# Fancomi2017/InstanceFusion

Hardware: AMD Instinct MI355X
Metric: frames/s + ms/frame (ICP|fuse|instance) at 640x480, 5M surfels, 1/2/4/8 GPU (higher is better)
Workload: dtype f32; 1 GPU; 5000000-surfel map, 640x480 synthetic RGBD stream, 3-level ICP+RGB + surfel fuse + canned-mask instance votes with superpixel refinement; surfels_live=4734799, surfel_slots=4734799, map_order=random, parallelism=replicas x1, loop_frames=90

## Files before the change

include/ifx_c_api.h:

```cpp
#ifndef IFX_C_API_H_
#define IFX_C_API_H_

#include <stdint.h>

#ifdef __cplusplus
extern "C" {
#endif

#define IFX_NUM_INSTANCES 96
#define IFX_VOTE_FLOATS 48

enum {
    IFX_OK = 0,
    IFX_E_INVALID = -1,
    IFX_E_HIP = -2,
    IFX_E_CAPACITY = -3,
    IFX_E_STATE = -4
};

typedef struct ifx_config {
    int32_t width, height;
    float fx, fy, cx, cy;
    int32_t time_delta;
    float confidence;
// ... 53 lines not shown
int ifx_owner_ids_resume(ifx_t* h);
int ifx_owner_knn_export(ifx_t* h, void** d_points, void** d_labels, int* n);
int ifx_owner_knn_vote(ifx_t* h, const void* d_all_points, const void* d_all_labels, int n_all, int own_offset);
int ifx_map_seq(ifx_t* h, uint32_t* out, int max_n);
int ifx_map_bounding_boxes(ifx_t* h, int bbox_type, float ratio, float* boxes96x6, float* ground_normal3, float* gc_matrix16, float* inst_matrix96x16,
                           int32_t* ground_votes648);
int ifx_instance_point_cloud(ifx_t* h, int bbox_type, int32_t* counts96, int inst, float* out10, int max_records);
int ifx_view_list_stats(ifx_t* h, int32_t* out4);
int ifx_sync(ifx_t* h);
int ifx_get_pose(ifx_t* h, float* out_pose16);
int ifx_tick(ifx_t* h);
int ifx_trajectory(ifx_t* h, float* out_poses16, int max_frames);
int ifx_tracker_diag(ifx_t* h, float* diag8);
int ifx_tracker_fallbacks(ifx_t* h);
int ifx_tracker_range_exceeded(ifx_t* h);

int ifx_set_loop_closure(ifx_t* h, int enable, int count_thresh, float err_thresh, float cov_thresh);
int ifx_loop_closure_diag(ifx_t* h, float* out24);
typedef int (*ifx_loop_closure_cb)(ifx_t* h, const float* lc24, void* user);
int ifx_set_loop_closure_callback(ifx_t* h, ifx_loop_closure_cb cb, void* user);
int ifx_sample_graph_model(ifx_t* h, float* out_xyzt, int max_n);
int ifx_loop_closure_constraints(ifx_t* h, float* src3, float* dst3, int32_t* times, int max_n);
int ifx_set_deformation(ifx_t* h, const float* graph16, int n_nodes, int is_fern);
int ifx_adopt_estimated_pose(ifx_t* h);

typedef int (*ifx_fern_cb)(ifx_t* h, void* user);
int ifx_set_fern_callback(ifx_t* h, ifx_fern_cb cb, void* user);
int ifx_adopt_pose(ifx_t* h, const float* pose16);
int ifx_fern_frame(ifx_t* h, uint8_t* img_rgb, float* verts4, float* norms4, uint8_t* inst_rgb);
int ifx_fern_frame_async(ifx_t* h);
// ... 184 lines not shown
```

instancefusion_amd/__init__.py:

```python
from __future__ import annotations

import ctypes as C
import functools
import os

import numpy as np

_HERE = os.path.dirname(os.path.abspath(__file__))
LIB_PATH = os.environ.get("IFX_LIB") or os.path.join(_HERE, "libifx.so")
HEADER_PATH = os.path.join(os.path.dirname(_HERE), "include", "ifx_c_api.h")

NUM_INSTANCES = 96
VOTE_FLOATS = 48


class IfxError(RuntimeError):
    pass


class IfxConfig(C.Structure):
    _fields_ = [
        ("width", C.c_int32), ("height", C.c_int32),
        ("fx", C.c_float), ("fy", C.c_float), ("cx", C.c_float), ("cy", C.c_float),
        ("time_delta", C.c_int32), ("confidence", C.c_float), ("depth_cut", C.c_float),
# ... 87 lines not shown
    "ifx_prefetch_frame_device": (C.c_int, [_P, _P, _P]),
    "ifx_hint_next_frame_device": (C.c_int, [_P, _P, _P]),
    "ifx_hint_next_frame": (C.c_int, [_P, _P, _P]),
    "ifx_lookahead_stats": (C.c_int, [_P, _P, C.c_int]),
    "ifx_view_list_stats": (C.c_int, [_P, _P]),
    "ifx_map_bounding_boxes": (C.c_int, [_P, C.c_int, C.c_float, _P, _P, _P, _P, _P]),
    "ifx_instance_point_cloud": (C.c_int, [_P, C.c_int, _P, C.c_int, _P, C.c_int]),
    "ifx_sync": (C.c_int, [_P]),
    "ifx_get_pose": (C.c_int, [_P, _P]),
    "ifx_tick": (C.c_int, [_P]),
    "ifx_trajectory": (C.c_int, [_P, _P, C.c_int]),
    "ifx_tracker_diag": (C.c_int, [_P, _P]),
    "ifx_tracker_fallbacks": (C.c_int, [_P]),
    "ifx_build_pyramids": (C.c_int, [_P, _P, _P, _P, _P, _P, _P, C.POINTER(Pyramids)]),
    "ifx_tracker_range_exceeded": (C.c_int, [_P]),
    "ifx_hot_records_stale": (C.c_int, [_P]),
    "ifx_set_loop_closure": (C.c_int, [_P, C.c_int, C.c_int, C.c_float, C.c_float]),
    "ifx_loop_closure_diag": (C.c_int, [_P, _P]),
    "ifx_set_loop_closure_callback": (C.c_int, [_P, _P, _P]),
    "ifx_sample_graph_model": (C.c_int, [_P, _P, C.c_int]),
    "ifx_loop_closure_constraints": (C.c_int, [_P, _P, _P, _P, C.c_int]),
    "ifx_set_deformation": (C.c_int, [_P, _P, C.c_int, C.c_int]),
    "ifx_adopt_estimated_pose": (C.c_int, [_P]),
    "ifx_set_fern_callback": (C.c_int, [_P, _P, _P]),
    "ifx_adopt_pose": (C.c_int, [_P, _P]),
    "ifx_fern_frame": (C.c_int, [_P, _P, _P, _P, _P]),
    "ifx_fern_frame_async": (C.c_int, [_P]),
    "ifx_fern_frame_fetch": (C.c_int, [_P, _P, _P, _P, _P]),
    "ifx_track_maps": (C.c_int, [_P, _P, _P, _P, _P, _P, _P, _P, _P]),
    "ifx_map_view": (C.c_int, [_P, C.POINTER(SoaView)]),
# ... 814 lines not shown
        out = np.zeros((max_frames, 16), np.float32)
        n = self._chk(self.L.ifx_trajectory(self.handle, _ptr(out), max_frames), "ifx_trajectory")
        return out[:n].reshape(n, 4, 4).copy()

    def tracker_diag(self):
        out = np.zeros(8, np.float32)
        self._chk(self.L.ifx_tracker_diag(self.handle, _ptr(out)), "ifx_tracker_diag")
        return out

    def tracker_fallbacks(self):
        return self._chk(self.L.ifx_tracker_fallbacks(self.handle), "ifx_tracker_fallbacks")

    def tracker_range_exceeded(self):
        return self._chk(self.L.ifx_tracker_range_exceeded(self.handle), "ifx_tracker_range_exceeded")

    def set_loop_closure(self, enable=True, count_thresh=35000, err_thresh=5e-5, cov_thresh=1e-5):
        self._chk(self.L.ifx_set_loop_closure(self.handle, int(enable), int(count_thresh), err_thresh, cov_thresh), "ifx_set_loop_closure")

    def loop_closure_diag(self):
        out = np.zeros(24, np.float32)
        self._chk(self.L.ifx_loop_closure_diag(self.handle, _ptr(out)), "ifx_loop_closure_diag")
        return dict(ran=bool(out[0]), inactive_pixels=int(out[1]), icp_error=float(out[2]), icp_count=float(out[3]), cov_ok=bool(out[4]),
                    accepted=bool(out[5]), est_pose=out[6:22].reshape(4, 4).copy(), cov_max=float(out[22]), candidates=int(out[23]))

    def set_loop_closure_callback(self, fn):
        if fn is None:
            self._lc_cb = None
            self._chk(self.L.ifx_set_loop_closure_callback(self.handle, None, None), "ifx_set_loop_closure_callback")
            return

# ... 481 lines not shown
```

instancefusion_amd/csrc/ifx_api.hip:

```cpp
#include <climits>
#include "ifx_ctx.h"
#include <string.h>
#include <stdio.h>
#include <algorithm>

int ifx_tracker_external_pose(ifx* h, const float* d_pose16, float weight_mult);
int ifx_tracker_set_weight(ifx* h, float weight_mult);
int ifx_compact_enqueue(ifx* h, int refresh_ids);

void hs_invalidate_view(ifx* h);
static std::string g_err;
extern "C" const char* ifx_global_error(void) { return g_err.c_str(); }
extern "C" const char* ifx_last_error(ifx_t* h) { return h ? h->err.c_str() : g_err.c_str(); }

hipEvent_t ifx_event_get(ifx* h)
{
    if (!h->event_pool.empty()) { hipEvent_t e = h->event_pool.back(); h->event_pool.pop_back(); return e; }
    hipEvent_t e;
    hipEventCreate(&e);
    return e;
}
void ifx_ktime_begin(ifx* h, const char* name, hipEvent_t* a)
{
    (void)name;
// ... 338 lines not shown
    else if (s == "ff_rounds") h->opt_ff_rounds = value;
    else if (s == "gn_persist_blocks") { if (value < 1) return IFX_E_INVALID; ifx_drop_tracked(h); h->opt_gn_persist_blocks = value; }
    else if (s == "gn_persist") {
        if (value < 0 || value > 7) { h->err = "gn_persist is a mask of pyramid levels (0..7)"; return IFX_E_INVALID; }
        ifx_drop_tracked(h);
        h->opt_gn_persist = value;
    }
    else if (s == "gn_spin_limit" || s == "gn_fault") {
        if (value < 0) return IFX_E_INVALID;
        ifx_drop_tracked(h);
        HIPCHK(h, hipStreamSynchronize(h->stream));
        HIPCHK(h, hipMemcpy((char*)h->d_state + (s == "gn_fault" ? offsetof(DevState, gn_fault) : offsetof(DevState, gn_spin_limit)), &value, sizeof(int), hipMemcpyHostToDevice));
    }
    else if (s == "gn_prologue") { ifx_drop_tracked(h); h->opt_gn_prologue = value ? 1 : 0; }
    else if (s == "rgb_cand") { ifx_drop_tracked(h); h->opt_rgb_cand = value ? 1 : 0; }
    else if (s == "raster_lds") h->opt_raster_lds = value;
    else if (s == "raster_earlyz") h->opt_raster_earlyz = value;
    else if (s == "pyramid" || s == "fast_odom" || s == "so3" || s == "icp_weight_x1000") {
        if (h->hint_rgb || h->slot[h->tick & 1].for_tick == h->tick) { h->err = "tracker options cannot change while a frame is announced ahead"; return IFX_E_STATE; }
        ifx_drop_tracked(h);
        if (s == "pyramid") h->cfg.pyramid = value ? 1 : 0;
        else if (s == "fast_odom") h->cfg.fast_odom = value ? 1 : 0;
        else if (s == "so3") h->cfg.so3 = value ? 1 : 0;
        else { if (value < 0 || value > 100000) { h->err = "icp_weight_x1000 must be in [0, 100000]"; return IFX_E_INVALID; } h->cfg.icp_weight = value / 1000.f; }
    }
    else { h->err = "unknown option " + s; return IFX_E_INVALID; }
    return IFX_OK;
}

__global__ void k_frame_result(DevState* __restrict__ st, FrameResult* __restrict__ out, float* __restrict__ traj_slot)
// ... 765 lines not shown
extern "C" int ifx_tracker_fallbacks(ifx_t* h)
{
    if (!h) return IFX_E_INVALID;
    int r = ifx_sync(h);
    return r ? r : h->h_result->gn_timeout;
}

extern "C" int ifx_hot_records_stale(ifx_t* h)
{
    if (!h) return IFX_E_INVALID;
    HIPCHK(h, hipStreamSynchronize(h->stream));
    int v = 0;
    HIPCHK(h, hipMemcpy(&v, &h->d_state->hot_stale, sizeof(int), hipMemcpyDeviceToHost));
    return v;
}
extern "C" int ifx_tracker_range_exceeded(ifx_t* h)
{
    if (!h) return IFX_E_INVALID;
    int r = ifx_sync(h);
    if (r) return r;
    if (h->stream_c) HIPCHK(h, hipStreamSynchronize(h->stream_c));
    if (h->stream_b) HIPCHK(h, hipStreamSynchronize(h->stream_b));
    std::vector<const DevState*> sts;
    sts.push_back(h->d_state);
    if (h->d_m2m) sts.push_back(h->d_m2m);
    if (h->d_cam_trk) sts.push_back(h->d_cam_trk);
    for (const FrameSlot& f : h->slot) if (f.so3) sts.push_back(f.so3);
    long long total = 0;
    for (const DevState* d : sts) {
        int v = 0;
// ... 396 lines not shown
```

instancefusion_amd/csrc/ifx_ctx.h:

```cpp
#pragma once
#include <hip/hip_runtime.h>
#include <stdint.h>
#include <string>
#include <vector>
#include <map>
#include "../../include/ifx_c_api.h"
#include "ifx_dev.h"

#ifndef IFX_LIST_SEGS
#define IFX_LIST_SEGS 8
#endif

struct DevState {
    float pose[16];
    float pose_inv[16];
    float last_pose[16];
    float weighting;
    int dense_enough;
    int count;
    int n_dead;
    int n_new;
    int overflow;
    unsigned int r_max_bits;
    float Rprev[9], tprev[3], Rprev_inv[9];
// ... 30 lines not shown
    int vl_scans;
    unsigned int vl_n[2];
    unsigned int vl_seg_n[2 * IFX_LIST_SEGS], vl_seg_off[2 * IFX_LIST_SEGS];
    long long dbg[8];
    alignas(64) int gn_res[2];
    unsigned int gn_ticket;
    int gn_pad[13];
    double gn_acc[2 * IFX_ACC_REPL * IFX_ACC_STRIDE];
    double gn_acc2[2 * 2 * IFX_ACC_REPL * IFX_ACC_STRIDE];
    alignas(64) int gn_res2[2 * 16];
    alignas(64) unsigned int gn_bar[4 * 32 * 16];
    int gn_timeout;
    int gn_abort;
    int gn_done_seq;
    int gn_spin_limit, gn_fault;
    alignas(64) double gnp_acc[2 * 2 * IFX_ACC_REPL * IFX_ACC_STRIDE];
    alignas(64) int gnp_res[2 * 16];
    alignas(64) double gnp_RRt[2][16];
};

struct IdMap { const uint32_t* seq; int own_n; };
__device__ __forceinline__ int idmap_slot(const IdMap& m, int count, int id)
{
    if (m.own_n <= 0) return (id > 0 && id < count) ? id : -1;
    if (id == 0) return -1;
    int lo = 0, hi = count - 1;
    while (lo <= hi) {
        const int mid = (lo + hi) >> 1;
        const unsigned int v = m.seq[mid];
        if (v == (unsigned int)id) return mid;
        if (v < (unsigned int)id) lo = mid + 1; else hi = mid - 1;
    }
    return -1;
// ... 228 lines not shown
    std::vector<int> oseg_cmp, oseg_bbox, oseg_class;
    hipEvent_t oseg_ev = nullptr;
    int32_t* oseg_rec = nullptr;
    size_t oseg_rec_cap = 0, oseg_rec_bytes = 0;
    int oseg_root = -1, oseg_form = 0, oseg_M = 0, oseg_maxn = 0;
    float oseg_thr = 0.f;
    const char* oseg_who = "";
    void* d_kexp = nullptr;
    int gn_begin_folded = 0;
    int labels_stale_all = 1;
    int opt_raster_lds = 0;
    int opt_view_blocks = 0, opt_clean_blocks = 0, opt_index_blocks = 0;
    int icp_resident_blocks = 1024;
    int opt_res_blocks = 0;
    int opt_rgb_cand = 1;
    int opt_icp_blocks = 0;
    int opt_raster_tiles = -1;
    int map_external = 0;
    int lc_enable = 0, lc_count_thresh = 35000;
    float lc_err_thresh = 5e-5f, lc_cov_thresh = 1e-5f;
    DevState* d_m2m = nullptr;
    Pyr m2m;
    float *old_vertex = nullptr, *old_normal = nullptr;
    uint8_t *old_image = nullptr, *old_inst = nullptr;
    uint16_t* old_time = nullptr;
    float *act_vertex = nullptr, *act_normal = nullptr;
    uint8_t *act_image = nullptr, *act_inst = nullptr;
    uint16_t* act_time = nullptr;
    size_t lc_half = 0;
    int own_tracked_tick = 0;
// ... 206 lines not shown
```

instancefusion_amd/csrc/ifx_track.hip:

```cpp
#include "ifx_ctx.h"
#include <math.h>
#include <string.h>


#define BIL_R 6
#define BIL_BX 32
#define BIL_BY 8
template <bool SHIFTED, bool XCLIP>
__device__ __forceinline__ void bil_window(const uint16_t (*tile)[BIL_BX + 2 * BIL_R + 3], const unsigned char* s_mapx, const unsigned char* s_mapy, int x, int y, int bx, int by, int tx1,
                                           int ty1, unsigned int value, float& sum1, float& sum2)
{
    const float ss = 0.024691358f, sc = 0.000555556f;
    constexpr int D = BIL_R * 2 + 1;
    const float fv = (float)value;
    for (int cy = max(y - D / 2, 0); cy < ty1; ++cy) {
        const int ry = SHIFTED ? (int)s_mapy[cy - by + BIL_R + 1] : cy - by + BIL_R + 1;
        const float dy = (float)y - (float)cy, dy2 = dy * dy;
        float tv[D];
#pragma unroll
        for (int q = 0; q < D; q++) {
            const int col = x - D / 2 + q - bx + BIL_R + 1;
            tv[q] = (float)tile[ry][SHIFTED ? (int)s_mapx[col] : col];
        }
#pragma unroll
// ... 333 lines not shown
            const float g = c_gauss25[(ty - cy - 1) * 5 + (tx - cx - 1)];
            const float sf = din[cy * sw + cx];
            if (!(sf != sf)) { sumf += sf * g; cntf += (int)g; }
            const int si = iin[cy * sw + cx];
            if (si > 0) { sumi += si * g; cnti += (int)g; }
        }
    const float z = (float)(sumf / (float)cntf);
    o.depth[y * dw + x] = z;
    o.img[y * dw + x] = cnti ? (uint8_t)f2i_rz(sumi / (float)cnti) : (uint8_t)0;
    model_tail(st, x, y, dw, dh, res[0], res[1], z, o);
}


#define RED_THREADS 256
#define RED_WAVES (RED_THREADS / 64)

__device__ __forceinline__ double dpp_quad_sum_d(double v)
{
    {
        const int lo = __builtin_amdgcn_update_dpp(0, __double2loint(v), 0xB1, 0xF, 0xF, true), hi = __builtin_amdgcn_update_dpp(0, __double2hiint(v), 0xB1, 0xF, 0xF, true);
        v += __hiloint2double(hi, lo);
    }
    {
        const int lo = __builtin_amdgcn_update_dpp(0, __double2loint(v), 0x4E, 0xF, 0xF, true), hi = __builtin_amdgcn_update_dpp(0, __double2hiint(v), 0x4E, 0xF, 0xF, true);
        v += __hiloint2double(hi, lo);
    }
    return v;
}
template <int NV>
__device__ __forceinline__ void block_sum_exact(const double* acc, double* __restrict__ gacc, int rep)
// ... 95 lines not shown

struct KInv { double i0, i4, i2, i5; };
struct GnPro {
    int k;
    int icp, rgb;
    float icp_weight;
    float nfx, nfy, ncx, ncy;
    KInv ki;
};
__device__ __forceinline__ void gn_serial_lane(const double* s_sys, int icp, double* RRt, const float* Rp, const float* tp, float nfx, float nfy, float ncx, float ncy, const KInv& ki,
                                               float* Rc, float* tc, float* krk, float* kt);
__device__ __forceinline__ const float* gn_prologue(const DevState* __restrict__ st, const GnPro& g, double* __restrict__ rrt_out)
{
    __shared__ double s_psys[27];
    __shared__ float s_ppose[24];
    const int prev = (g.k - 1) & 1;
    const double* const icp_acc = st->gnp_acc + (size_t)(prev * 2) * IFX_ACC_REPL * IFX_ACC_STRIDE;
    const double* const rgb_acc = icp_acc + IFX_ACC_REPL * IFX_ACC_STRIDE;
    if (threadIdx.x < 27) {
        const int k = threadIdx.x;
        const double ti = acc_total(icp_acc, k), tr = acc_total(rgb_acc, k);
        const float oi = g.icp ? (float)ti : 0.f, orr = g.rgb ? (float)tr : 0.f;
        const double wgt = g.icp_weight;
        const double wa = wgt * wgt, wb = wgt;
        const bool is_b = (k == 6) | (k == 12) | (k == 17) | (k == 21) | (k == 24) | (k == 26);
        const double vi = (double)oi, vr = (double)orr;
        s_psys[k] = (g.icp && g.rgb) ? vr + (is_b ? wb : wa) * vi : (g.icp ? vi : vr);
    }
    const double* const rsrc = g.k == 1 ? st->resultRt : st->gnp_RRt[g.k & 1];
    double RRt[16];
    float Rp[9], tp[3];
// ... 195 lines not shown
        int s = 0;
        for (int wv = 0; wv < RED_WAVES; wv++) s += lds[wv][threadIdx.x];
        if (!FROM_STATE) partials[bid * 2 + threadIdx.x] = s;
        if (res_total && s) atomicAdd(&res_total[threadIdx.x], s);
    }
}
__global__ __launch_bounds__(RED_THREADS) void k_rgb_residual(const DevState* __restrict__ st, ResArgs ex, float minScale, const int16_t* __restrict__ dIdx,
                                                              const int16_t* __restrict__ dIdy, const float* __restrict__ lastDepth,
                                                              const float* __restrict__ nextDepth, const uint8_t* __restrict__ lastImage,
                                                              const uint8_t* __restrict__ nextImage, Corres8* __restrict__ corres, float maxDepthDelta,
                                                              int w, int h, int* __restrict__ partials)
{
    residual_body(blockIdx.x, gridDim.x, st, ex, minScale, dIdx, dIdy, lastDepth, nextDepth, lastImage, nextImage, corres, maxDepthDelta, w, h, partials);
}

template <bool PRO>
__device__ __forceinline__ void residual_cand_body(int bid, int nblk, const DevState* __restrict__ st, const CandEntry* __restrict__ cand, const unsigned int* __restrict__ cand_n,
                                                   const float* __restrict__ lastDepth, const float* __restrict__ nextDepth, const uint8_t* __restrict__ lastImage,
                                                   const uint8_t* __restrict__ nextImage, Corres8* __restrict__ corres, float maxDepthDelta, int w, int h,
                                                   int* __restrict__ res_total, const GnPro* pro, double* __restrict__ rrt_out)
{
    const int N = w * h;
    const int stride = nblk * RED_THREADS;
    int t = bid * RED_THREADS + threadIdx.x;
    const int n = min((int)cand_n[0], N);
    const CandEntry e0 = cand[t < N ? t : 0];
    CandEntry e1 = cand[t + stride < N ? t + stride : 0];
    int pix = t < n ? (int)min(e0.pixel, (uint32_t)(N - 1)) : 0;
    float d1 = nextDepth[pix];
    uint8_t ni = nextImage[pix];
    const float* kk = st->krkinv;
    const float* ktp = st->kt;
    if (PRO) { const float* sp = gn_prologue(st, *pro, rrt_out); kk = sp + 12; ktp = sp + 21; }
    float krk[9];
#pragma unroll
    for (int k = 0; k < 9; k++) krk[k] = kk[k];
    const float kt0 = ktp[0], kt1 = ktp[1], kt2 = ktp[2];
    int cnt = 0, sig = 0;
    while (t < n) {
        const int i = pix / w, j0 = pix - i * w;
// ... 5 lines not shown
        const int gj = c0 ? v0 * w + u0 : 0;
        const float d0 = lastDepth[gj];
        const uint8_t li = lastImage[gj];
        const int tn = t + stride, tnn = tn + stride;
        const int pixn = tn < n ? (int)min(e1.pixel, (uint32_t)(N - 1)) : 0;
        const float d1n = nextDepth[pixn];
        const uint8_t nin = nextImage[pixn];
        const CandEntry e2 = cand[tnn < N ? tnn : 0];
        Corres8 c;
        const bool hit = c0 & (d0 > 0) & (fabsf(td1 - d0) <= maxDepthDelta) & (li != 0);
        const float diff = (float)ni - (float)li;
        c.zx = hit ? (short)u0 : (short)-1; c.zy = hit ? (short)v0 : (short)-1;
        c.diff = hit ? diff : 0.f;
        cnt += hit ? 1 : 0;
        sig += hit ? (int)(diff * diff) : 0;
        corres[t] = c;
        t = tn; pix = pixn; d1 = d1n; ni = nin; e1 = e2;
    }
    __shared__ int lds[RED_WAVES][2];
    const int lane = threadIdx.x & 63, wid = threadIdx.x >> 6;
    cnt = wave_sum_i(cnt);
    sig = wave_sum_i(sig);
    if (lane == 0) { lds[wid][0] = cnt; lds[wid][1] = sig; }
    __syncthreads();
    if (threadIdx.x < 2) {
        int s = 0;
        for (int wv = 0; wv < RED_WAVES; wv++) s += lds[wv][threadIdx.x];
        if (s) atomicAdd(&res_total[threadIdx.x], s);
    }
}

struct PairArgs {
    const float *vmap_curr, *nmap_curr, *vmap_prev, *nmap_prev;
    float fx, fy, cx, cy, distThres, angleThres;
    float minScale, maxDepthDelta;
    const int16_t *dIdx, *dIdy;
    const float *lastDepth, *nextDepth;
    const uint8_t *lastImage, *nextImage;
    Corres8* corres;
    int w, h, nb_icp, nb_res;
    int check_skip;
};
#define IFX_PIN_S(x) asm volatile("" ::"s"(x))
template <bool CHECK_SKIP, bool PRO = false, bool LIST = false>
__global__ __launch_bounds__(RED_THREADS, 4) void k_icp_residual(const DevState* __restrict__ st, int nb_icp, int w, int h, double* __restrict__ gacc, int* __restrict__ gres, PairArgs a, GnPro g,
                                                              double* __restrict__ rrt_store, const CandEntry* __restrict__ cand, const unsigned int* __restrict__ cand_n)
{
    __builtin_assume(st != nullptr);
    if (CHECK_SKIP && st->skip) return;
    if ((int)blockIdx.x < nb_icp) {
        IcpArgs ia;
        icp_body<false, true, PRO>(blockIdx.x, nb_icp, st, ia, a.vmap_curr, a.nmap_curr, a.vmap_prev, a.nmap_prev, a.fx, a.fy, a.cx, a.cy, a.distThres, a.angleThres, w, h, gacc, &g,
                                   blockIdx.x == 0 ? rrt_store : nullptr);
    } else if (LIST) {
        residual_cand_body<PRO>(blockIdx.x - nb_icp, a.nb_res, st, cand, cand_n, a.lastDepth, a.nextDepth, a.lastImage, a.nextImage, a.corres, a.maxDepthDelta, w, h, gres, &g,
                                blockIdx.x == 0 ? rrt_store : nullptr);
    } else {
        ResArgs ra;
        residual_body<true, PRO>(blockIdx.x - nb_icp, a.nb_res, st, ra, a.minScale, a.dIdx, a.dIdy, a.lastDepth, a.nextDepth, a.lastImage, a.nextImage, a.corres, a.maxDepthDelta, w,
                                 h, nullptr, gres, &g, blockIdx.x == 0 ? rrt_store : nullptr);
    }
}
// ... 915 lines not shown
    int icp, rgb;
    float icp_weight, nfx, nfy, ncx, ncy;
    KInv ki;
    int check_skip;
    int final_iter;
    int end_run, commit;
    float weight_mult;
    unsigned int* lctr;
    int pro, pro_k;
};
template <bool CHECK_SKIP, bool LIST = false>
__global__ __launch_bounds__(RED_THREADS) void k_rgb_step_solve(DevState* st, int nb, int rgb, int w, int h, StepArgs a, const CandEntry* __restrict__ cand, const unsigned int* __restrict__ cand_n)
{
    __builtin_assume(st != nullptr);
    if (CHECK_SKIP && st->skip) return;
    const int par = a.pro_k & 1;
    int* const res_total = a.pro ? st->gnp_res + par * 16 : st->gn_res;
    unsigned int* const ticket = &st->gn_ticket;
    double* const icp_acc = a.pro ? st->gnp_acc + (size_t)(par * 2) * IFX_ACC_REPL * IFX_ACC_STRIDE : st->gn_acc;
    double* const rgb_acc = icp_acc + IFX_ACC_REPL * IFX_ACC_STRIDE;
    __shared__ int s_last;
    if (a.pro && blockIdx.x == 0) {
        double* const other = st->gnp_acc + (size_t)((1 - par) * 2) * IFX_ACC_REPL * IFX_ACC_STRIDE;
        if (threadIdx.x < 64) {
            const int kind = threadIdx.x >> 5, k = threadIdx.x & 31;
            if (k < 28 && range_exceeded7(kind, k, acc_total(other + (size_t)kind * IFX_ACC_REPL * IFX_ACC_STRIDE, k))) atomicAdd(&st->range_exceeded, 1);
        }
        __syncthreads();
        __hip_atomic_store(&other[threadIdx.x], 0.0, __ATOMIC_RELAXED, __HIP_MEMORY_SCOPE_AGENT);
        if (threadIdx.x < 2) __hip_atomic_store(&st->gnp_res[(1 - par) * 16 + threadIdx.x], 0, __ATOMIC_RELAXED, __HIP_MEMORY_SCOPE_AGENT);
    }
#ifdef IFX_STAMPS
    long long t0 = clock64();
#endif
    if (rgb) {
        if (LIST) rgb_step_cand_body(blockIdx.x, nb, a.corres, cand, cand_n, a.cloud, a.fx, a.fy, a.sobelScale, w, h, rgb_acc, res_total);
        else rgb_step_body(blockIdx.x, nb, a.corres, 0.f, nullptr, 0, a.cloud, a.fx, a.fy, a.dIdx, a.dIdy, a.sobelScale, w, h, rgb_acc, res_total);
    }
    if (a.pro == 1) return;
    asm volatile("s_waitcnt vmcnt(0)" ::: "memory");
    __syncthreads();
#ifdef IFX_STAMPS
    long long t1 = clock64();
#endif
    if (threadIdx.x == 0) {
// ... 497 lines not shown
    const int maxb = 1024;
    HIPCHK(h, hipMalloc(&p.acc, (3 * IFX_ACC_REPL * IFX_ACC_STRIDE * sizeof(double))));
    HIPCHK(h, hipMemset(p.acc, 0, (3 * IFX_ACC_REPL * IFX_ACC_STRIDE * sizeof(double))));
    {
        int cus = 0, dev = 0;
        hipGetDevice(&dev);
        hipDeviceGetAttribute(&cus, hipDeviceAttributeMultiprocessorCount, dev);
        int occ[4] = {0, 0, 0, 0};
        hipOccupancyMaxActiveBlocksPerMultiprocessor(&occ[0], k_gn_level<1>, RED_THREADS, 0);
        hipOccupancyMaxActiveBlocksPerMultiprocessor(&occ[1], k_gn_level<2>, RED_THREADS, 0);
        hipOccupancyMaxActiveBlocksPerMultiprocessor(&occ[2], k_gn_level<3>, RED_THREADS, 0);
        hipOccupancyMaxActiveBlocksPerMultiprocessor(&occ[3], k_gn_level<4>, RED_THREADS, 0);
        for (int q = 0; q < 4; q++) h->gn_max_blocks[q] = std::max(0, occ[q]) * std::max(0, cus);
        int occ_ir = 0;
        if (hipOccupancyMaxActiveBlocksPerMultiprocessor(&occ_ir, k_icp_residual<false, true>, RED_THREADS, 0) == hipSuccess && occ_ir > 0 && cus > 0) h->icp_resident_blocks = occ_ir * cus;
    }
    h->res_rows = std::max(maxb, cdiv(h->P, RED_THREADS) + 1);
    HIPCHK(h, hipMalloc(&h->res_partials, (size_t)h->res_rows * 2 * 4));
    HIPCHK(h, hipMalloc(&h->d_out29, 64 * 4));
    HIPCHK(h, hipMalloc(&h->d_ticket, 512));
    HIPCHK(h, hipMemset(h->d_ticket, 0, 512));
    p.res_partials = h->res_partials; p.ticket = h->d_ticket;
    for (int q = 0; q < 2; q++) {
        HIPCHK(h, hipMalloc(&h->slot[q].so3, sizeof(DevState)));
        HIPCHK(h, hipMemset(h->slot[q].so3, 0, sizeof(DevState)));
    }
    ifx_bind_slot(h, 0);
    return IFX_OK;
}

// ... 29 lines not shown
        hipFree(h->d_cam_trk); hipFree(h->cam_so3_acc); hipFree(h->cam_so3_ticket);
        h->d_cam_trk = nullptr;
    }
    free_m2m(h);
    hipFree(h->d_graph); hipFree(h->d_sample); hipFree(h->d_cons); hipFree(h->d_project); hipFree(h->d_fern); hipFree(h->d_inst_gt);
    if (h->h_fern) hipHostFree(h->h_fern);
    if (h->ev_fern) hipEventDestroy(h->ev_fern);
    hipFree(h->pyr.acc); hipFree(h->res_partials); hipFree(h->d_out29); hipFree(h->d_ticket);
}

static inline int rgb_cand_blocks(const ifx* h, int n, int level, bool step)
{
    const int per_thread = 8 >> std::min(level, 2), opt = step ? h->opt_rgb_blocks : h->opt_res_blocks;
    const int b = opt > 0 ? std::min(opt, cdiv(n, RED_THREADS)) : cdiv(n, RED_THREADS * per_thread * (step ? RED_IT_RGB : 1));
    return std::max(1, b);
}
static inline int red_blocks(ifx* h, int n, int it = RED_IT)
{
    int b = cdiv(n, RED_THREADS * it);
    const int cap = h->opt_icp_blocks > 0 ? h->opt_icp_blocks : std::max(456, std::min(1024, h->P / 2048));
    if (b > cap) b = cap;
    if (b < 1) b = 1;
    return b;
}

int ifx_tracker_init_first(ifx* h)
{
    Pyr& p = h->pyr;
    LAUNCH(h, "intensity", dim3(cdiv(h->P, 256)), dim3(256), k_intensity, h->rgb, 3, h->P, p.lastnext_img[0]);
    for (int i = 0; i + 1 < IFX_NUM_PYRS; i++)
// ... 175 lines not shown
            if (iterations[i] <= 0) continue;
            if (persist_q[i] >= 0) { if (seen_two_launch) pro = false; }
            else {
                seen_two_launch = true;
                const int n = p.w[i] * p.h[i];
                const int blocks = (icp ? red_blocks(h, n) : 0) + (cand_run ? rgb_cand_blocks(h, n, i, false) : rgb ? std::min(std::min(cdiv(n, RED_THREADS * RED_IT), h->res_rows), h->opt_res_blocks > 0 ? h->opt_res_blocks : (1 << 30)) : 0);
                small = small && blocks <= h->opt_gn_prologue_blocks;
                if (small) n_pro += iterations[i];
            }
        }
        if (n_pro < 2) pro = false;
    }
    int persist_iters = 0;
    int tail_k = 0;
    char* const stb = (char*)st;
    auto gnp_acc_of = [&](int par) { return (double*)(stb + offsetof(DevState, gnp_acc)) + (size_t)(par * 2) * IFX_ACC_REPL * IFX_ACC_STRIDE; };
    auto gnp_res_of = [&](int par) { return (int*)(stb + offsetof(DevState, gnp_res)) + par * 16; };
    auto gnp_rrt_of = [&](int par) { return (double*)(stb + offsetof(DevState, gnp_RRt)) + par * 16; };
    static const char* const icp_name[3] = {"icp_residual@L0", "icp_residual@L1", "icp_residual@L2"};
    static const char* const rgb_name[3] = {"rgb_step_solve@L0", "rgb_step_solve@L1", "rgb_step_solve@L2"};
    static_assert(IFX_NUM_PYRS == 3, "level names");
    for (int i = IFX_NUM_PYRS - 1; i >= 0; i--) {
        if (i == 0 && frame_tracker) ifx_enqueue_hinted_frame_side(h);
        float div = (float)(1 << i);
        float fx = c.fx / div, fy = c.fy / div, cx = c.cx / div, cy = c.cy / div;
        int lw = p.w[i], lh = p.h[i], n = lw * lh, nb = red_blocks(h, n), nb_rgb = cand_run ? rgb_cand_blocks(h, n, i, true) : std::min(red_blocks(h, n, RED_IT_RGB), h->opt_rgb_blocks > 0 ? h->opt_rgb_blocks : 192);
        const float ld = next_div[i];
        PairArgs pa = pair_args(i);
        const int res_round = std::max(128, h->icp_resident_blocks - (icp ? nb : 0));
        const int nbr = cand_run ? rgb_cand_blocks(h, n, i, false) : std::min(std::min(cdiv(n, RED_THREADS * RED_IT), h->res_rows), h->opt_res_blocks > 0 ? h->opt_res_blocks : res_round);
        const CandEntry* const cl = cand_run ? p.cand[i] : nullptr;
        const unsigned int* const cln = cand_run ? p.cand_n[i] : nullptr;
// ... 13 lines not shown
            persist_iters += iterations[i];
            la.final_level = finer[i] ? 0 : 1; la.commit = commit; la.weight_mult = weight_mult; la.lctr = frame_tracker ? h->d_list_ctr : (unsigned int*)nullptr;
            auto go = [&](auto kernel) { LAUNCH(h, "gn_level", dim3(nbp), dim3(RED_THREADS), kernel, st, la); };
            if (q == 0) go(k_gn_level<1>);
            else if (q == 1) go(k_gn_level<2>);
            else if (q == 2) go(k_gn_level<3>);
            else go(k_gn_level<4>);
            LAUNCH(h, "gn_level_solo", dim3(1), dim3(RED_THREADS), k_gn_level_solo, st, la);
            ended = ended || la.final_level;
            continue;
        }
        for (int j = 0; j < iterations[i]; j++) {
            GnPro gp;
            gp.k = tail_k; gp.icp = icp; gp.rgb = rgb; gp.icp_weight = icp_weight; gp.nfx = fx; gp.nfy = fy; gp.ncx = cx; gp.ncy = cy; gp.ki = kinv_of(fx, fy, cx, cy);
            const bool it_pro = pro && tail_k < n_pro;
            double* const ga = it_pro ? gnp_acc_of(tail_k & 1) : gacc;
            int* const gr = it_pro ? gnp_res_of(tail_k & 1) : gres;
            double* const rrt_store = gnp_rrt_of((tail_k + 1) & 1);
            auto go_icp = [&](auto kernel) { LAUNCH(h, icp_name[i], dim3(pa.nb_icp + pa.nb_res), dim3(RED_THREADS), kernel, st, pa.nb_icp, pa.w, pa.h, ga, gr, pa, gp, rrt_store, cl, cln); };
            if (it_pro && tail_k > 0) {
                if (frame_tracker) { if (cand_run) go_icp(k_icp_residual<false, true, true>); else go_icp(k_icp_residual<false, true>); }
                else { if (cand_run) go_icp(k_icp_residual<true, true, true>); else go_icp(k_icp_residual<true, true>); }
            } else {
                if (frame_tracker) { if (cand_run) go_icp(k_icp_residual<false, false, true>); else go_icp(k_icp_residual<false, false>); }
                else { if (cand_run) go_icp(k_icp_residual<true, false, true>); else go_icp(k_icp_residual<true, false>); }
            }
            StepArgs sa2 = step_args(i, j);
            sa2.nb = nb_rgb; sa2.nb_icp = nb; sa2.nb_res = nbr; sa2.check_skip = frame_tracker ? 0 : 1; sa2.lctr = frame_tracker ? h->d_list_ctr : (unsigned int*)nullptr;
            sa2.pro = (pro && tail_k < n_pro) ? (tail_k == n_pro - 1 ? 2 : 1) : 0; sa2.pro_k = tail_k;
            tail_k++;
            ended = ended || sa2.end_run;
            auto go_rgb = [&](auto kernel) { LAUNCH(h, rgb_name[i], dim3(nb_rgb), dim3(RED_THREADS), kernel, st, sa2.nb, sa2.rgb, sa2.w, sa2.h, sa2, cl, cln); };
            if (frame_tracker) { if (cand_run) go_rgb(k_rgb_step_solve<false, true>); else go_rgb(k_rgb_step_solve<false>); }
            else { if (cand_run) go_rgb(k_rgb_step_solve<true, true>); else go_rgb(k_rgb_step_solve<true>); }
// ... 551 lines not shown
```

Baseline: 1688 frames/s.

## Fuse photometric GN step into residual kernel via in-kernel grid meet

Adds a fused path where the residual kernel's RGB blocks, after writing correspondences, meet at a global counter and then accumulate the photometric normal-equation rows in work-stolen chunks. This removes the separate rgb_step_solve launch per Gauss-Newton iteration. The prologue accumulators move to a three-set rotation so the clear of the next set can happen inside the fused kernel. In exchange, the RGB work runs on a small fixed block count and relies on a bounded spin-wait that can give up, with a counter exposed to report give-ups.

```diff
diff --git a/include/ifx_c_api.h b/include/ifx_c_api.h
--- a/include/ifx_c_api.h
+++ b/include/ifx_c_api.h
@@ -91,6 +91,7 @@
 int ifx_tracker_diag(ifx_t* h, float* diag8);
 int ifx_tracker_fallbacks(ifx_t* h);
 int ifx_tracker_range_exceeded(ifx_t* h);
+int ifx_tracker_meet_giveups(ifx_t* h);
 
 int ifx_set_loop_closure(ifx_t* h, int enable, int count_thresh, float err_thresh, float cov_thresh);
 int ifx_loop_closure_diag(ifx_t* h, float* out24);
diff --git a/instancefusion_amd/__init__.py b/instancefusion_amd/__init__.py
--- a/instancefusion_amd/__init__.py
+++ b/instancefusion_amd/__init__.py
@@ -125,6 +125,7 @@
     "ifx_tracker_fallbacks": (C.c_int, [_P]),
     "ifx_build_pyramids": (C.c_int, [_P, _P, _P, _P, _P, _P, _P, C.POINTER(Pyramids)]),
     "ifx_tracker_range_exceeded": (C.c_int, [_P]),
+    "ifx_tracker_meet_giveups": (C.c_int, [_P]),
     "ifx_hot_records_stale": (C.c_int, [_P]),
     "ifx_set_loop_closure": (C.c_int, [_P, C.c_int, C.c_int, C.c_float, C.c_float]),
     "ifx_loop_closure_diag": (C.c_int, [_P, _P]),
@@ -969,6 +970,9 @@
     def tracker_range_exceeded(self):
         return self._chk(self.L.ifx_tracker_range_exceeded(self.handle), "ifx_tracker_range_exceeded")
 
+    def tracker_meet_giveups(self):
+        return self._chk(self.L.ifx_tracker_meet_giveups(self.handle), "ifx_tracker_meet_giveups")
+
     def set_loop_closure(self, enable=True, count_thresh=35000, err_thresh=5e-5, cov_thresh=1e-5):
         self._chk(self.L.ifx_set_loop_closure(self.handle, int(enable), int(count_thresh), err_thresh, cov_thresh), "ifx_set_loop_closure")
 
diff --git a/instancefusion_amd/csrc/ifx_api.hip b/instancefusion_amd/csrc/ifx_api.hip
--- a/instancefusion_amd/csrc/ifx_api.hip
+++ b/instancefusion_amd/csrc/ifx_api.hip
@@ -376,6 +376,12 @@
     }
     else if (s == "gn_prologue") { ifx_drop_tracked(h); h->opt_gn_prologue = value ? 1 : 0; }
     else if (s == "rgb_cand") { ifx_drop_tracked(h); h->opt_rgb_cand = value ? 1 : 0; }
+    else if (s == "rgb_fuse") {
+        if (value < 0 || value > 7) { h->err = "rgb_fuse is a mask of pyramid levels (0..7)"; return IFX_E_INVALID; }
+        ifx_drop_tracked(h);
+        h->opt_rgb_fuse = value;
+    }
+    else if (s == "rgb_fuse_poll") { ifx_drop_tracked(h); h->opt_rgb_fuse_poll = value ? 1 : 0; }
     else if (s == "raster_lds") h->opt_raster_lds = value;
     else if (s == "raster_earlyz") h->opt_raster_earlyz = value;
     else if (s == "pyramid" || s == "fast_odom" || s == "so3" || s == "icp_weight_x1000") {
@@ -1171,6 +1177,22 @@
     HIPCHK(h, hipMemcpy(&v, &h->d_state->hot_stale, sizeof(int), hipMemcpyDeviceToHost));
     return v;
 }
+extern "C" int ifx_tracker_meet_giveups(ifx_t* h)
+{
+    if (!h) return IFX_E_INVALID;
+    int r = ifx_sync(h);
+    if (r) return r;
+    if (h->stream_c) HIPCHK(h, hipStreamSynchronize(h->stream_c));
+    if (h->stream_b) HIPCHK(h, hipStreamSynchronize(h->stream_b));
+    long long total = 0;
+    for (const DevState* d : {(const DevState*)h->d_state, (const DevState*)h->d_cam_trk}) {
+        if (!d) continue;
+        int v = 0;
+        HIPCHK(h, hipMemcpy(&v, (const char*)d + offsetof(DevState, rgb_meet_giveups), sizeof(int), hipMemcpyDeviceToHost));
+        total += v;
+    }
+    return (int)std::min<long long>(total, 0x7FFFFFFF);
+}
 extern "C" int ifx_tracker_range_exceeded(ifx_t* h)
 {
     if (!h) return IFX_E_INVALID;
diff --git a/instancefusion_amd/csrc/ifx_ctx.h b/instancefusion_amd/csrc/ifx_ctx.h
--- a/instancefusion_amd/csrc/ifx_ctx.h
+++ b/instancefusion_amd/csrc/ifx_ctx.h
@@ -68,9 +68,11 @@
     int gn_abort;
     int gn_done_seq;
     int gn_spin_limit, gn_fault;
-    alignas(64) double gnp_acc[2 * 2 * IFX_ACC_REPL * IFX_ACC_STRIDE];
-    alignas(64) int gnp_res[2 * 16];
+    alignas(64) double gnp_acc[3 * 2 * IFX_ACC_REPL * IFX_ACC_STRIDE];
+    alignas(64) int gnp_res[3 * 16];
+    alignas(64) unsigned int gnp_meet[3 * 32];
     alignas(64) double gnp_RRt[2][16];
+    int rgb_meet_giveups;
 };
 
 struct IdMap { const uint32_t* seq; int own_n; };
@@ -329,6 +331,9 @@
     int icp_resident_blocks = 1024;
     int opt_res_blocks = 0;
     int opt_rgb_cand = 1;
+    int opt_rgb_fuse = 7;
+    int opt_rgb_fuse_poll = 1;
+    int icp_resident_blocks_fuse = 1024;
     int opt_icp_blocks = 0;
     int opt_raster_tiles = -1;
     int map_external = 0;
diff --git a/instancefusion_amd/csrc/ifx_rgb_chunks.h b/instancefusion_amd/csrc/ifx_rgb_chunks.h
--- /dev/null
+++ b/instancefusion_amd/csrc/ifx_rgb_chunks.h
@@ -0,0 +1,29 @@
+#pragma once
+
+#if defined(__HIPCC__) || defined(__CUDACC__)
+#define IFX_HD __host__ __device__
+#else
+#define IFX_HD
+#endif
+
+#define RGB_CHUNK_THREADS 256
+#define RGB_CHUNK_IT 2
+#define RGB_CHUNK (RGB_CHUNK_THREADS * RGB_CHUNK_IT)
+
+struct RgbChunk { int first, end; };
+
+IFX_HD inline int rgb_chunk_n(unsigned int cand_n, int capacity)
+{
+    const unsigned int cap = capacity > 0 ? (unsigned int)capacity : 0u;
+    return (int)(cand_n < cap ? cand_n : cap);
+}
+IFX_HD inline int rgb_chunk_count(int n) { return n <= 0 ? 0 : (n - 1) / RGB_CHUNK + 1; }
+IFX_HD inline RgbChunk rgb_chunk_range(unsigned int chunk, int n)
+{
+    RgbChunk r;
+    const unsigned int count = (unsigned int)rgb_chunk_count(n);
+    if (chunk >= count) { r.first = n > 0 ? n : 0; r.end = r.first; return r; }
+    r.first = (int)chunk * RGB_CHUNK;
+    r.end = n - r.first < RGB_CHUNK ? n : r.first + RGB_CHUNK;
+    return r;
+}
diff --git a/instancefusion_amd/csrc/ifx_track.hip b/instancefusion_amd/csrc/ifx_track.hip
--- a/instancefusion_amd/csrc/ifx_track.hip
+++ b/instancefusion_amd/csrc/ifx_track.hip
@@ -1,4 +1,5 @@
 #include "ifx_ctx.h"
+#include "ifx_rgb_chunks.h"
 #include <math.h>
 #include <string.h>
 
@@ -371,6 +372,7 @@
 
 #define RED_THREADS 256
 #define RED_WAVES (RED_THREADS / 64)
+static_assert(RGB_CHUNK_THREADS == RED_THREADS, "a chunk of the fused photometric step is RGB_CHUNK_IT records per thread of a reduction block");
 
 __device__ __forceinline__ double dpp_quad_sum_d(double v)
 {
@@ -496,7 +498,7 @@
 {
     __shared__ double s_psys[27];
     __shared__ float s_ppose[24];
-    const int prev = (g.k - 1) & 1;
+    const int prev = (g.k - 1) % 3;
     const double* const icp_acc = st->gnp_acc + (size_t)(prev * 2) * IFX_ACC_REPL * IFX_ACC_STRIDE;
     const double* const rgb_acc = icp_acc + IFX_ACC_REPL * IFX_ACC_STRIDE;
     if (threadIdx.x < 27) {
@@ -722,8 +724,8 @@
     residual_body(blockIdx.x, gridDim.x, st, ex, minScale, dIdx, dIdy, lastDepth, nextDepth, lastImage, nextImage, corres, maxDepthDelta, w, h, partials);
 }
 
-template <bool PRO>
-__device__ __forceinline__ void residual_cand_body(int bid, int nblk, const DevState* __restrict__ st, const CandEntry* __restrict__ cand, const unsigned int* __restrict__ cand_n,
+template <bool PRO, bool SC1 = false>
+__device__ __forceinline__ int residual_cand_body(int bid, int nblk, const DevState* __restrict__ st, const CandEntry* __restrict__ cand, const unsigned int* __restrict__ cand_n,
                                                    const float* __restrict__ lastDepth, const float* __restrict__ nextDepth, const uint8_t* __restrict__ lastImage,
                                                    const uint8_t* __restrict__ nextImage, Corres8* __restrict__ corres, float maxDepthDelta, int w, int h,
                                                    int* __restrict__ res_total, const GnPro* pro, double* __restrict__ rrt_out)
@@ -731,7 +733,7 @@
     const int N = w * h;
     const int stride = nblk * RED_THREADS;
     int t = bid * RED_THREADS + threadIdx.x;
-    const int n = min((int)cand_n[0], N);
+    const int n = SC1 ? rgb_chunk_n(cand_n[0], N) : min((int)cand_n[0], N);
     const CandEntry e0 = cand[t < N ? t : 0];
     CandEntry e1 = cand[t + stride < N ? t + stride : 0];
     int pix = t < n ? (int)min(e0.pixel, (uint32_t)(N - 1)) : 0;
@@ -767,7 +769,11 @@
         c.diff = hit ? diff : 0.f;
         cnt += hit ? 1 : 0;
         sig += hit ? (int)(diff * diff) : 0;
-        corres[t] = c;
+        if (SC1) {
+            unsigned long long bits;
+            __builtin_memcpy(&bits, &c, 8);
+            __hip_atomic_store(reinterpret_cast<unsigned long long*>(corres + t), bits, __ATOMIC_RELAXED, __HIP_MEMORY_SCOPE_AGENT);
+        } else corres[t] = c;
         t = tn; pix = pixn; d1 = d1n; ni = nin; e1 = e2;
     }
     __shared__ int lds[RED_WAVES][2];
@@ -781,6 +787,125 @@
         for (int wv = 0; wv < RED_WAVES; wv++) s += lds[wv][threadIdx.x];
         if (s) atomicAdd(&res_total[threadIdx.x], s);
     }
+    return n;
+}
+
+#define RGB_MEET_TICKS 5372u
+struct FuseArgs {
+    const float* cloud;
+    float sobelScale;
+    int g;
+    unsigned int poll_ticks;
+    unsigned int* meet;
+    double* clear_acc;
+    int* clear_res;
+    unsigned int* clear_meet;
+    int* range_ctr;
+    int* giveups;
+};
+static_assert(sizeof(Corres8) == 8, "a record is handed over as one 8-byte store");
+__device__ __forceinline__ void gnp_clear_set(double* acc, int* res, unsigned int* meet, int* range_ctr)
+{
+    if (threadIdx.x < 64) {
+        const int kind = threadIdx.x >> 5, k = threadIdx.x & 31;
+        if (k < 28 && range_exceeded7(kind, k, acc_total(acc + (size_t)kind * IFX_ACC_REPL * IFX_ACC_STRIDE, k))) atomicAdd(range_ctr, 1);
+    }
+    __syncthreads();
+    static_assert(2 * IFX_ACC_REPL * IFX_ACC_STRIDE == RED_THREADS, "one store per thread clears a set's rows");
+    __hip_atomic_store(&acc[threadIdx.x], 0.0, __ATOMIC_RELAXED, __HIP_MEMORY_SCOPE_AGENT);
+    if (threadIdx.x < 2) __hip_atomic_store(&res[threadIdx.x], 0, __ATOMIC_RELAXED, __HIP_MEMORY_SCOPE_AGENT);
+    if (threadIdx.x >= 64 && threadIdx.x < 66) __hip_atomic_store(&meet[(threadIdx.x - 64) * 16], 0u, __ATOMIC_RELAXED, __HIP_MEMORY_SCOPE_AGENT);
+}
+__device__ __forceinline__ void rgb_fused_step(int bid, int n_wave, Corres8* corres, const CandEntry* __restrict__ cand, int w, int h, float fx, float fy, int* res_total,
+                                               double* __restrict__ rgb_acc, const FuseArgs& f)
+{
+    __shared__ int s_go, s_n;
+    __shared__ unsigned int s_chunk;
+    asm volatile("s_waitcnt vmcnt(0)" ::: "memory");
+    __syncthreads();
+    if (threadIdx.x == 0) {
+        const unsigned int all = (unsigned int)f.g;
+        const unsigned int t = __hip_atomic_fetch_add(&f.meet[0], 1u, __ATOMIC_RELAXED, __HIP_MEMORY_SCOPE_AGENT);
+        int go = t + 1u >= all;
+        if (!go) {
+            if (f.poll_ticks) {
+                const unsigned long long t0 = wall_clock64();
+                for (;;) {
+                    if (__hip_atomic_load(&f.meet[0], __ATOMIC_RELAXED, __HIP_MEMORY_SCOPE_AGENT) >= all) { go = 1; break; }
+                    if (wall_clock64() - t0 > (unsigned long long)f.poll_ticks) break;
+                    __builtin_amdgcn_s_sleep(2);
+                }
+            }
+            if (!go) atomicAdd(f.giveups, 1);
+        }
+        s_chunk = go ? __hip_atomic_fetch_add(&f.meet[16], 1u, __ATOMIC_RELAXED, __HIP_MEMORY_SCOPE_AGENT) : 0xFFFFFFFFu;
+        s_go = go;
+        s_n = n_wave;
+    }
+    __syncthreads();
+    if (!s_go) return;
+    const int n = __builtin_amdgcn_readfirstlane(s_n);
+    unsigned int chunk = s_chunk;
+    if (chunk >= (unsigned int)rgb_chunk_count(n)) return;
+    float sigma;
+    {
+        const int cnt = __hip_atomic_load(&res_total[0], __ATOMIC_RELAXED, __HIP_MEMORY_SCOPE_AGENT), sg = __hip_atomic_load(&res_total[1], __ATOMIC_RELAXED, __HIP_MEMORY_SCOPE_AGENT);
+        float q = (float)sg / (float)cnt;
+        sigma = (float)sqrt((double)((q == 0) ? 1 : cnt));
+    }
+    double acc[29];
+#pragma unroll
+    for (int k = 0; k < 29; k++) acc[k] = 0.0;
+    for (;;) {
+        const RgbChunk r = rgb_chunk_range(chunk, n);
+        if (r.first >= r.end) break;
+        Corres8 c[RGB_CHUNK_IT];
+        CandEntry e[RGB_CHUNK_IT];
+#pragma unroll
+        for (int u = 0; u < RGB_CHUNK_IT; u++) {
+            const int k = r.first + (int)threadIdx.x + u * RED_THREADS;
+            const bool in = k < r.end;
+            const int kk = in ? k : r.first;
+            const unsigned long long bits = __hip_atomic_load(reinterpret_cast<unsigned long long*>(corres + kk), __ATOMIC_RELAXED, __HIP_MEMORY_SCOPE_AGENT);
+            __builtin_memcpy(&c[u], &bits, 8);
+            e[u] = cand[kk];
+            if (!in) c[u].zx = -1;
+        }
+        __syncthreads();
+        if (threadIdx.x == 0) s_chunk = __hip_atomic_fetch_add(&f.meet[16], 1u, __ATOMIC_RELAXED, __HIP_MEMORY_SCOPE_AGENT);
+        float X[RGB_CHUNK_IT], Y[RGB_CHUNK_IT], Z[RGB_CHUNK_IT];
+#pragma unroll
+        for (int u = 0; u < RGB_CHUNK_IT; u++) {
+            if (!((c[u].zx >= 0) & (c[u].zx < w) & (c[u].zy >= 0) & (c[u].zy < h))) c[u].zx = -1;
+            int g = (c[u].zx >= 0) ? ((int)c[u].zy * w + (int)c[u].zx) * 3 : 0;
+            X[u] = f.cloud[g]; Y[u] = f.cloud[g + 1]; Z[u] = f.cloud[g + 2];
+        }
+#pragma unroll
+        for (int u = 0; u < RGB_CHUNK_IT; u++) {
+            float row[7] = {0, 0, 0, 0, 0, 0, 0};
+            bool found = c[u].zx >= 0;
+            if (found) {
+                float wgt = sigma + fabsf(c[u].diff);
+                wgt = wgt > 1.19209290E-07F ? 1.0f / wgt : 1.0f;
+                if (sigma == -1) wgt = 1;
+                row[6] = -wgt * c[u].diff;
+                float invz = (float)(1.0 / Z[u]);
+                float dI_dx = wgt * f.sobelScale * e[u].gx;
+                float dI_dy = wgt * f.sobelScale * e[u].gy;
+                float v0 = dI_dx * fx * invz;
+                float v1 = dI_dy * fy * invz;
+                float v2 = -(v0 * X[u] + v1 * Y[u]) * invz;
+                row[0] = v0; row[1] = v1; row[2] = v2;
+                row[3] = -Z[u] * v1 + Y[u] * v2;
+                row[4] = Z[u] * v0 - X[u] * v2;
+                row[5] = -Y[u] * v0 + X[u] * v1;
+            }
+            products7<1>(row, found, acc);
+        }
+        __syncthreads();
+        chunk = s_chunk;
+    }
+    block_sum_exact<29>(acc, rgb_acc, bid % IFX_ACC_REPL);
 }
 
 struct PairArgs {
@@ -795,10 +920,27 @@
     int check_skip;
 };
 #define IFX_PIN_S(x) asm volatile("" ::"s"(x))
-template <bool CHECK_SKIP, bool PRO = false, bool LIST = false>
+template <bool CHECK_SKIP, bool PRO = false, bool LIST = false, bool FUSE = false>
 __global__ __launch_bounds__(RED_THREADS, 4) void k_icp_residual(const DevState* __restrict__ st, int nb_icp, int w, int h, double* __restrict__ gacc, int* __restrict__ gres, PairArgs a, GnPro g,
-                                                              double* __restrict__ rrt_store, const CandEntry* __restrict__ cand, const unsigned int* __restrict__ cand_n)
-{
+                                                              double* __restrict__ rrt_store, const CandEntry* __restrict__ cand, const unsigned int* __restrict__ cand_n, FuseArgs f)
+{
+    static_assert(!FUSE || LIST, "the fused iteration runs over the candidate list");
+    if (FUSE) {
+        __builtin_assume(st != nullptr);
+        if (CHECK_SKIP && st->skip) return;
+        const int nb_rgb = (int)gridDim.x - nb_icp;
+        if (blockIdx.x == gridDim.x - 1) gnp_clear_set(f.clear_acc, f.clear_res, f.clear_meet, f.range_ctr);
+        if ((int)blockIdx.x < nb_rgb) {
+            const int n = residual_cand_body<PRO, true>(blockIdx.x, nb_rgb, st, cand, cand_n, a.lastDepth, a.nextDepth, a.lastImage, a.nextImage, a.corres, a.maxDepthDelta, w, h, gres, &g,
+                                                        blockIdx.x == 0 ? rrt_store : nullptr);
+            rgb_fused_step(blockIdx.x, n, a.corres, cand, w, h, a.fx, a.fy, gres, gacc + IFX_ACC_REPL * IFX_ACC_STRIDE, f);
+        } else {
+            IcpArgs ia;
+            icp_body<false, true, PRO>(blockIdx.x - nb_rgb, nb_icp, st, ia, a.vmap_curr, a.nmap_curr, a.vmap_prev, a.nmap_prev, a.fx, a.fy, a.cx, a.cy, a.distThres, a.angleThres, w, h, gacc, &g,
+                                       blockIdx.x == 0 ? rrt_store : nullptr);
+        }
+        return;
+    }
     __builtin_assume(st != nullptr);
     if (CHECK_SKIP && st->skip) return;
     if ((int)blockIdx.x < nb_icp) {
@@ -1744,21 +1886,17 @@
 {
     __builtin_assume(st != nullptr);
     if (CHECK_SKIP && st->skip) return;
-    const int par = a.pro_k & 1;
-    int* const res_total = a.pro ? st->gnp_res + par * 16 : st->gn_res;
+    const int par = a.pro_k & 1, set = a.pro_k % 3;
+    int* const res_total = a.pro ? st->gnp_res + set * 16 : st->gn_res;
     unsigned int* const ticket = &st->gn_ticket;
-    double* const icp_acc = a.pro ? st->gnp_acc + (size_t)(par * 2) * IFX_ACC_REPL * IFX_ACC_STRIDE : st->gn_acc;
+    double* const icp_acc = a.pro ? st->gnp_acc + (size_t)(set * 2) * IFX_ACC_REPL * IFX_ACC_STRIDE : st->gn_acc;
     double* const rgb_acc = icp_acc + IFX_ACC_REPL * IFX_ACC_STRIDE;
     __shared__ int s_last;
     if (a.pro && blockIdx.x == 0) {
-        double* const other = st->gnp_acc + (size_t)((1 - par) * 2) * IFX_ACC_REPL * IFX_ACC_STRIDE;
-        if (threadIdx.x < 64) {
-            const int kind = threadIdx.x >> 5, k = threadIdx.x & 31;
-            if (k < 28 && range_exceeded7(kind, k, acc_total(other + (size_t)kind * IFX_ACC_REPL * IFX_ACC_STRIDE, k))) atomicAdd(&st->range_exceeded, 1);
-        }
-        __syncthreads();
-        __hip_atomic_store(&other[threadIdx.x], 0.0, __ATOMIC_RELAXED, __HIP_MEMORY_SCOPE_AGENT);
-        if (threadIdx.x < 2) __hip_atomic_store(&st->gnp_res[(1 - par) * 16 + threadIdx.x], 0, __ATOMIC_RELAXED, __HIP_MEMORY_SCOPE_AGENT);
+        for (int d = 1; d <= (a.pro == 2 ? 2 : 1); d++) {
+            const int cs = (a.pro_k + d) % 3;
+            gnp_clear_set(st->gnp_acc + (size_t)(cs * 2) * IFX_ACC_REPL * IFX_ACC_STRIDE, st->gnp_res + cs * 16, st->gnp_meet + cs * 32, &st->range_exceeded);
+        }
     }
 #ifdef IFX_STAMPS
     long long t0 = clock64();
@@ -2286,6 +2424,8 @@
         for (int q = 0; q < 4; q++) h->gn_max_blocks[q] = std::max(0, occ[q]) * std::max(0, cus);
         int occ_ir = 0;
         if (hipOccupancyMaxActiveBlocksPerMultiprocessor(&occ_ir, k_icp_residual<false, true>, RED_THREADS, 0) == hipSuccess && occ_ir > 0 && cus > 0) h->icp_resident_blocks = occ_ir * cus;
+        int occ_fu = 0;
+        if (hipOccupancyMaxActiveBlocksPerMultiprocessor(&occ_fu, k_icp_residual<false, true, true, true>, RED_THREADS, 0) == hipSuccess && occ_fu > 0 && cus > 0) h->icp_resident_blocks_fuse = occ_fu * cus;
     }
     h->res_rows = std::max(maxb, cdiv(h->P, RED_THREADS) + 1);
     HIPCHK(h, hipMalloc(&h->res_partials, (size_t)h->res_rows * 2 * 4));
@@ -2345,6 +2485,11 @@
     const int per_thread = 8 >> std::min(level, 2), opt = step ? h->opt_rgb_blocks : h->opt_res_blocks;
     const int b = opt > 0 ? std::min(opt, cdiv(n, RED_THREADS)) : cdiv(n, RED_THREADS * per_thread * (step ? RED_IT_RGB : 1));
     return std::max(1, b);
+}
+#define RGB_FUSE_BLOCKS 32
+static inline int rgb_fuse_blocks(const ifx* h, int n)
+{
+    return std::max(1, std::min(h->opt_rgb_blocks > 0 ? h->opt_rgb_blocks : RGB_FUSE_BLOCKS, cdiv(n, RED_THREADS)));
 }
 static inline int red_blocks(ifx* h, int n, int it = RED_IT)
 {
@@ -2550,8 +2695,9 @@
     int persist_iters = 0;
     int tail_k = 0;
     char* const stb = (char*)st;
-    auto gnp_acc_of = [&](int par) { return (double*)(stb + offsetof(DevState, gnp_acc)) + (size_t)(par * 2) * IFX_ACC_REPL * IFX_ACC_STRIDE; };
-    auto gnp_res_of = [&](int par) { return (int*)(stb + offsetof(DevState, gnp_res)) + par * 16; };
+    auto gnp_acc_of = [&](int set) { return (double*)(stb + offsetof(DevState, gnp_acc)) + (size_t)(set * 2) * IFX_ACC_REPL * IFX_ACC_STRIDE; };
+    auto gnp_res_of = [&](int set) { return (int*)(stb + offsetof(DevState, gnp_res)) + set * 16; };
+    auto gnp_meet_of = [&](int set) { return (unsigned int*)(stb + offsetof(DevState, gnp_meet)) + set * 32; };
     auto gnp_rrt_of = [&](int par) { return (double*)(stb + offsetof(DevState, gnp_RRt)) + par * 16; };
     static const char* const icp_name[3] = {"icp_residual@L0", "icp_residual@L1", "icp_residual@L2"};
     static const char* const rgb_name[3] = {"rgb_step_solve@L0", "rgb_step_solve@L1", "rgb_step_solve@L2"};
@@ -2595,10 +2741,27 @@
             GnPro gp;
             gp.k = tail_k; gp.icp = icp; gp.rgb = rgb; gp.icp_weight = icp_weight; gp.nfx = fx; gp.nfy = fy; gp.ncx = cx; gp.ncy = cy; gp.ki = kinv_of(fx, fy, cx, cy);
             const bool it_pro = pro && tail_k < n_pro;
-            double* const ga = it_pro ? gnp_acc_of(tail_k & 1) : gacc;
-            int* const gr = it_pro ? gnp_res_of(tail_k & 1) : gres;
+            const bool fuse = cand_run && it_pro && tail_k < n_pro - 1 && (h->opt_rgb_fuse & (1 << i));
+            double* const ga = it_pro ? gnp_acc_of(tail_k % 3) : gacc;
+            int* const gr = it_pro ? gnp_res_of(tail_k % 3) : gres;
             double* const rrt_store = gnp_rrt_of((tail_k + 1) & 1);
-            auto go_icp = [&](auto kernel) { LAUNCH(h, icp_name[i], dim3(pa.nb_icp + pa.nb_res), dim3(RED_THREADS), kernel, st, pa.nb_icp, pa.w, pa.h, ga, gr, pa, gp, rrt_store, cl, cln); };
+            FuseArgs fa;
+            memset(&fa, 0, sizeof(fa));
+            PairArgs paf = pa;
+            if (fuse) {
+                paf.nb_res = std::max(1, std::min(rgb_fuse_blocks(h, n), h->icp_resident_blocks_fuse - pa.nb_icp));
+                const int cs = (tail_k + 1) % 3;
+                fa.cloud = p.cloud[i]; fa.sobelScale = (float)sobelScale; fa.g = paf.nb_res; fa.poll_ticks = h->opt_rgb_fuse_poll ? RGB_MEET_TICKS : 0u;
+                fa.meet = gnp_meet_of(tail_k % 3); fa.clear_acc = gnp_acc_of(cs); fa.clear_res = gnp_res_of(cs); fa.clear_meet = gnp_meet_of(cs);
+                fa.range_ctr = (int*)(stb + offsetof(DevState, range_exceeded)); fa.giveups = (int*)(stb + offsetof(DevState, rgb_meet_giveups));
+            }
+            auto go_icp = [&](auto kernel) { LAUNCH(h, icp_name[i], dim3(paf.nb_icp + paf.nb_res), dim3(RED_THREADS), kernel, st, paf.nb_icp, paf.w, paf.h, ga, gr, paf, gp, rrt_store, cl, cln, fa); };
+            if (fuse) {
+                if (tail_k > 0) { if (frame_tracker) go_icp(k_icp_residual<false, true, true, true>); else go_icp(k_icp_residual<true, true, true, true>); }
+                else { if (frame_tracker) go_icp(k_icp_residual<false, false, true, true>); else go_icp(k_icp_residual<true, false, true, true>); }
+                tail_k++;
+                continue;
+            }
             if (it_pro && tail_k > 0) {
                 if (frame_tracker) { if (cand_run) go_icp(k_icp_residual<false, true, true>); else go_icp(k_icp_residual<false, true>); }
                 else { if (cand_run) go_icp(k_icp_residual<true, true, true>); else go_icp(k_icp_residual<true, true>); }
```

Measured after the change: 1844 frames/s, median of 6. 1.09x the previous value.
